# jakub-zarzycki2022/gym-PBN-stac

Measured on NVIDIA B200. Metric: bittner100_env_steps_per_s, higher is better.
Workload: dtype u32

## Files before the change

### gym-pbn-stac_b200/csrc/pbn_b200.cu

```cuda
#include <cmath>
#include <cstdio>
#include <cstdlib>
#include <cstring>
#include <map>
#include <mutex>
#include <string>
#include <type_traits>
#include <vector>

#include "pbn_device.cuh"

static thread_local std::string g_err;
static int fail(int code, const std::string &msg) {
    g_err = msg;
    return code;
}
#define CK(call)                                                                                     \
    do {                                                                                             \
        cudaError_t e_ = (call);                                                                     \
        if (e_ != cudaSuccess) {                                                                     \
            cudaGetLastError();                                                                      \
            return fail(PBN_ERR_CUDA, std::string(#call) + ": " + cudaGetErrorString(e_));           \
        }                                                                                            \
    } while (0)
// ... 1274 lines not shown
    }
    vec_flush_stats(vx, s_stats);
}

template <int MODE>
__global__ void __launch_bounds__(PBN_BLOCK) k_rand_state(NetView nv, DrawView dv, u32 *state, long long B, long long env0) {
    const long long e = (long long)blockIdx.x * blockDim.x + threadIdx.x;
    if (e >= B) return;
    Draw<MODE> d;
    d.init(dv, e, env0 + e);
    u32 acc = 0;
    for (int i = 0; i < nv.n; i++) {
        acc |= (u32)d.randint(0, 2) << (i & 31);
        if ((i & 31) == 31 || i == nv.n - 1) { state[(long long)(i >> 5) * B + e] = acc; acc = 0; }
    }
    d.done(dv, e);
}

__global__ void __launch_bounds__(PBN_BLOCK) k_attractor_index(EnvView ev, int w32, const u32 *state, long long B, int *att_out,
                                                               int staged) {
    const unsigned char *img = staged ? smem_raw : ev.img;
    u32 *sst = reinterpret_cast<u32 *>(smem_raw + index_smem(ev, w32, staged).cols);
    if (staged) stage(smem_raw, ev.img, ev.img_bytes);
    const int *att_off = reinterpret_cast<const int *>(img);
    const u32 *cubes = reinterpret_cast<const u32 *>(img + ev.off_cubes);
    const long long e = (long long)blockIdx.x * PBN_BLOCK + threadIdx.x;
    Col st{sst + threadIdx.x};
    if (e < B) load_state(st, state, B, e, w32);
    __syncthreads();
    if (e >= B) return;
    int idx = -1;
    for (int a = 0; a < ev.n_att && idx < 0; a++)
        if (match_range(cubes, att_off[a], att_off[a + 1], st, w32)) idx = a;
    att_out[e] = idx;
}

__device__ __forceinline__ int ssd_bucket(const SsdParams &sp, const u32 *s_tgt, const Col &st) {
    if (sp.fast_t0 >= 0) {
        u32 field = (*st.wp((u32)sp.fast_t0) >> (sp.fast_t0 & 31)) << (32 - sp.g);
        return (int)__brev(field);
    }
    int b = 0;
    for (int k = 0; k < sp.g; k++) b = (b << 1) | (int)st.bit(s_tgt[k]);
    return b;
}

struct SsdLoopArgs {
    const NetView &nv;
    const EnvView &ev;
    const SsdParams &sp;
    const DrawView &dv;
    const unsigned char *blob;
    const int *att_off;
    const u32 *cubes;
    const u32 *s_tgt;
    u32 *shist;
    unsigned long long *hist;
    u32 *sst;
    int iters;
    u32 nvalid;
    u32 *flipbuf;
    int win;
    long long chain_id;
    unsigned char *coop_buf;
};

__device__ __forceinline__ u32 warp_scan_add(u32 v) {
#pragma unroll
    for (int off = 1; off < 32; off <<= 1)
        asm volatile("{ .reg .pred p; .reg .u32 t; shfl.sync.up.b32 t|p, %0, %1, 0, 0xffffffff; @p add.u32 %0, %0, t; }"
                     : "+r"(v) : "r"(off));
    return v;
}

struct SsdPerturb {
    u32 e0, e1;
    u32 last_p1;
};

__device__ __forceinline__ u32 ssd_gap(u32 word, float inv, float hmd) {
    bool ok;
    u32 gap = geom_gap_approx(word, inv, hmd, &ok);
    if (!ok) gap = geom_gap(word, inv);
    return gap;
}

__device__ __forceinline__ void ssd_round(SsdPerturb &ps, u32 g0, u32 g1) {
    const u32 incl = warp_scan_add(g0 + g1 + 2u);
    ps.e1 = ps.last_p1 - 1u + incl;
    ps.e0 = ps.e1 - 1u - g1;
    ps.last_p1 = __shfl_sync(0xFFFFFFFFu, ps.e1, 31) + 1u;
}

template <bool FULL>
__device__ __forceinline__ void ssd_perturb(SsdPerturb &ps, Draw<PBN_DRAW_PHILOX> &dp, char *warp_cols, u32 W, float inv, float hmd, u32 nvalid) {
    auto apply = [&](u32 &e) {
        if (e < W) {
            const u32 tl = e & 31u;
            if (FULL || tl < nvalid) atomicXor(reinterpret_cast<u32 *>(warp_cols + tl * 4u + ((e >> 10) << 10)), 1u << ((e >> 5) & 31u));
            e = 0xFFFFFFFFu;
        }
    };
    for (;;) {
        apply(ps.e0);
        apply(ps.e1);
        if (ps.last_p1 > W) break;
        const u32 g0 = ssd_gap(dp.next(), inv, hmd);
        const u32 g1 = ssd_gap(dp.next(), inv, hmd);
        ssd_round(ps, g0, g1);
    }
    if (ps.e0 != 0xFFFFFFFFu) ps.e0 -= W;
    if (ps.e1 != 0xFFFFFFFFu) ps.e1 -= W;
    ps.last_p1 -= W;
    __syncwarp();
}

template <bool FULL>
__device__ __forceinline__ void ssd_perturb_buf(SsdPerturb &ps, Draw<PBN_DRAW_PHILOX> &dp, u32 *buf, u32 W, float inv, float hmd, u32 nvalid) {
    auto apply = [&](u32 &e) {
        if (e < W) {
            const u32 tl = e & 31u;
            if (FULL || tl < nvalid) atomicXor(buf + ((e >> 10) << 5) + tl, 1u << ((e >> 5) & 31u));
            e = 0xFFFFFFFFu;
        }
    };
    for (;;) {
        apply(ps.e0);
        apply(ps.e1);
        if (ps.last_p1 > W) break;
        const u32 g0 = ssd_gap(dp.next(), inv, hmd);
        const u32 g1 = ssd_gap(dp.next(), inv, hmd);
        ssd_round(ps, g0, g1);
    }
    if (ps.e0 != 0xFFFFFFFFu) ps.e0 -= W;
    if (ps.e1 != 0xFFFFFFFFu) ps.e1 -= W;
    ps.last_p1 -= W;
}

struct SsdCount {
    int cur;
    u32 run;
};
__device__ __forceinline__ void ssd_count(SsdCount &c, const SsdLoopArgs &a, const Col &st) {
    const int b = ssd_bucket(a.sp, a.s_tgt, st);
    if (b != c.cur) {
        if (a.sp.smem_hist) atomicAdd(&a.shist[c.cur], c.run);
        else atomicAdd(&a.hist[c.cur], (unsigned long long)c.run);
        c.cur = b; c.run = 0;
    }
    c.run++;
}

struct SsdFastPerturb {
    u32 e0, e1, last_p1;
    u32 blk, half, sx, sy;
};

__device__ __forceinline__ void ssd_fast_apply(const SsdFast &f, u32 e) {
    asm volatile("{ .reg .pred p; setp.lt.u32 p, %0, %1; @p red.shared.xor.b32 [%2], %3; }"
                 :: "r"(e), "r"(f.W), "r"((f.warp_cols | ((e << 2) & 0x7Cu)) | (e & 0xFFFFFC00u)),
                    "r"(1u << ((e >> 5) & 31u)) : "memory");
}

__device__ __forceinline__ u32 ssd_fast_gap(const SsdFast &f, u32 word, bool &ok) { return geom_gap_approx(word, f.inv, f.gdelta, &ok); }

__device__ __forceinline__ void ssd_fast_perturb(const SsdFast &f, SsdFastPerturb &ps, const Draw<PBN_DRAW_PHILOX> &dp, const DrawView &dv) {
    ssd_fast_apply(f, ps.e0);
    ssd_fast_apply(f, ps.e1);
    while (ps.last_p1 <= f.W) {
        u32 wa, wb;
        if (ps.half == 0u) {
            u32 x2, x3;
            philox4x32_10_rk(ps.blk, dp.c1, dp.c2, dp.c3, dv, wa, wb, x2, x3);
            ps.blk++;
            ps.sx = x2; ps.sy = x3;
            ps.half = 1u;
        } else {
            wa = ps.sx; wb = ps.sy;
            ps.half = 0u;
        }
        bool ok0, ok1;
        u32 g0 = ssd_fast_gap(f, wa, ok0), g1 = ssd_fast_gap(f, wb, ok1);
        if (!(ok0 && ok1)) {
            if (!ok0) g0 = geom_gap(wa, f.inv);
            if (!ok1) g1 = geom_gap(wb, f.inv);
        }
        const u32 incl = warp_scan_add(g0 + g1 + 2u);
        ps.e1 = ps.last_p1 - 1u + incl;
        ps.e0 = ps.e1 - 1u - g1;
        ps.last_p1 = __reduce_max_sync(0xFFFFFFFFu, ps.e1) + 1u;
        ssd_fast_apply(f, ps.e0);
        ssd_fast_apply(f, ps.e1);
    }
    ps.e0 -= f.W;
    ps.e1 -= f.W;
    ps.last_p1 -= f.W;
    __syncwarp();
}

template <int TQ>
__device__ __forceinline__ int ssd_loop_pred_static(const SsdLoopArgs &a, const Col &st, Draw<PBN_DRAW_PHILOX> &d,
                                                    Draw<PBN_DRAW_PHILOX> &dp, SsdPerturb &ps0, SsdCount &cnt) {
    const NetView &nv = a.nv;
    SsdFast f;
    f.col = keep(smem_addr(st.s));
    f.warp_cols = keep(smem_addr(a.sst + (threadIdx.x & ~31u)));
    f.thr = keep(smem_addr(a.blob + nv.off_thr));
    f.rec = keep(smem_addr(a.blob + nv.off_rec16));
    f.thr_stride = keep((u32)nv.tsq_stride * 16u);
    f.rec_stride = keep((u32)nv.fmax * 16u);
    f.shist = keep(smem_addr(a.shist));
    f.n = keep((u32)nv.n);
    f.W = keep((u32)nv.n * 32u);
    f.b_off = keep(((u32)a.sp.fast_t0 >> 5) << 10);
    f.b_sh = keep((u32)a.sp.fast_t0 & 31u);
    f.b_up = keep(32u - (u32)a.sp.g);
    f.inv = a.sp.inv;
    f.gdelta = 0.5f - a.sp.gdelta;
    SsdFastPerturb ps{ps0.e0, ps0.e1, ps0.last_p1, dp.blk, 0u, 0u, 0u};
    u32 ublk = 0;
    int t = 0;
    u32 cur = (u32)cnt.cur, run = cnt.run;
    auto count = [&]() {
        const u32 b = __brev((lds_u32(f.col + f.b_off) >> f.b_sh) << f.b_up);
        u32 r0;
        asm volatile("{ .reg .pred p; setp.ne.u32 p, %1, %2; @p red.shared.add.u32 [%3], %4; selp.u32 %0, 0, %4, p; }"
                     : "=r"(r0) : "r"(b), "r"(cur), "r"(f.shist + cur * 4u), "r"(run) : "memory");
        cur = b;
        run = r0 + 1u;
    };
    for (int left = a.iters >> 1; left > 0; left--, t += 2) {
        u32 x0, x1, x2, x3;
        philox4x32_10_rk(ublk, d.c1, d.c2, d.c3, a.dv, x0, x1, x2, x3);
        ublk++;
        const FastDraw da = ssd_fast_draw<TQ>(f, x0, x1);
        count();
        ssd_fast_perturb(f, ps, dp, a.dv);
        ssd_fast_apply_update(f, da);
        __syncwarp();
        const FastDraw db = ssd_fast_draw<TQ>(f, x2, x3);
        count();
        ssd_fast_perturb(f, ps, dp, a.dv);
        ssd_fast_apply_update(f, db);
        __syncwarp();
    }
    d.blk = ublk;
    d.have = 0;
    dp.blk = ps.blk;
    dp.have = ps.half ? 2 : 0;
    dp.b0 = ps.sx; dp.b1 = ps.sy;
    ps0.e0 = ps.e0 >= 0x80000000u ? 0xFFFFFFFFu : ps.e0;
    ps0.e1 = ps.e1 >= 0x80000000u ? 0xFFFFFFFFu : ps.e1;
    ps0.last_p1 = ps.last_p1;
    cnt.cur = (int)cur; cnt.run = run;
    return t;
}

template <int NET, int MODE, int TQ, bool HAS_ENV, bool FULL>
__device__ __forceinline__ void ssd_loop(const SsdLoopArgs &a, const Col &st, Draw<MODE> &d, Draw<MODE> &dp) {
    const NetView &nv = a.nv;
    const SsdParams &sp = a.sp;
    const u32 lane = threadIdx.x & 31u;
    const bool active = FULL || lane < a.nvalid;
    const u32 n = (u32)nv.n, W = n * 32u;
    const float inv = sp.inv;
    const float hmd = 0.5f - sp.gdelta;
    const bool flips = inv <= 0.f;
    SsdPerturb ps{0xFFFFFFFFu, 0xFFFFFFFFu, 0u};
    char *warp_cols = reinterpret_cast<char *>(a.sst + (threadIdx.x & ~31u));
    SsdCount cnt{active ? ssd_bucket(sp, a.s_tgt, st) : 0, 0u};
    int t = 0;
    if constexpr (MODE == PBN_DRAW_PHILOX && !HAS_ENV && FULL && NET == PBN_NET_PRED && TQ > 0) {
        if (flips && sp.smem_hist && sp.fast_t0 >= 0 && nv.off_rec16) t = ssd_loop_pred_static<TQ>(a, st, d, dp, ps, cnt);
    }
    if constexpr (MODE == PBN_DRAW_PHILOX && !HAS_ENV && FULL) {
        u32 ublk = d.blk;
        for (; t + 1 < a.iters; t += 2) {
            u32 x0, x1, x2, x3;
            philox4x32_10(ublk, d.c1, d.c2, d.c3, d.k0, d.k1, x0, x1, x2, x3);
            ublk++;
            ssd_count(cnt, a, st);
            if (flips) ssd_perturb<true>(ps, dp, warp_cols, W, inv, hmd, 32u);
            micro_step_words<NET, TQ>(nv, a.blob, st, x0, x1, d);
            __syncwarp();
            ssd_count(cnt, a, st);
            if (flips) ssd_perturb<true>(ps, dp, warp_cols, W, inv, hmd, 32u);
            micro_step_words<NET, TQ>(nv, a.blob, st, x2, x3, d);
            __syncwarp();
        }
        d.blk = ublk;
        d.have = 0;
    }
    if constexpr (MODE == PBN_DRAW_PHILOX && HAS_ENV) {
        if (a.flipbuf != nullptr && !a.ev.force) {
            const int w32 = nv.w32;
            u32 *fb = a.flipbuf + (size_t)(threadIdx.x >> 5) * a.win * w32 * 32;
            u32 pos = 0;
            while (t < a.iters) {
                const int kk = a.iters - t < a.win ? a.iters - t : a.win;
                for (int k = 0; k < kk; k++) {
                    for (int w = 0; w < w32; w++) fb[(k * w32 + w) * 32 + lane] = 0u;
                    __syncwarp();
                    if (flips) ssd_perturb_buf<FULL>(ps, dp, fb + k * w32 * 32, W, inv, hmd, a.nvalid);
                }
                __syncwarp();
                int k = 0, in = 0;
                bool start = true;
                for (;;) {
                    const bool live = active && k < kk;
                    if (!__any_sync(0xFFFFFFFFu, live)) break;
                    if (live) {
                        if (start) {
                            ssd_count(cnt, a, st);
                            for (int w = 0; w < w32; w++) st.set_word(w, st.word(w) ^ fb[(k * w32 + w) * 32 + lane]);
                            micro_step<NET, MODE, TQ>(nv, a.blob, st, d);
                            in = 1;
                            pos++;
                            start = false;
                        } else if (in >= a.ev.max_inner || is_attracting(a.ev, a.att_off, a.cubes, st, w32)) {
                            k++;
                            start = true;
                        } else {
                            micro_step<NET, MODE, TQ>(nv, a.blob, st, d);
                            in++;
                            pos++;
                        }
                    }
                    if constexpr (NET == PBN_NET_PRED) {
                        const unsigned hv = __ballot_sync(0xFFFFFFFFu, live && !start && k < kk);
                        if (hv != 0u && __popc(__ballot_sync(0xFFFFFFFFu, active && k < kk)) <= PBN_COOP_MAX) {
                            const u32 base = pos - (u32)in;
                            const int v = w32 == 1 ? coop_take_over<TQ, true>(hv, nv, a.ev, a.dv, a.blob, a.att_off, a.cubes, a.sst, a.coop_buf,
                                                                              a.chain_id, in, base, a.ev.max_inner, 32)
                                                   : coop_take_over<TQ, false>(hv, nv, a.ev, a.dv, a.blob, a.att_off, a.cubes, a.sst, a.coop_buf,
                                                                               a.chain_id, in, base, a.ev.max_inner, 32);
                            if (v != in) {
                                pos += (u32)(v - in);
                                in = v;
                                d.seek(a.dv, 0, a.chain_id, 2u * pos, 0u);
                            }
                        }
                    }
                }
                __syncwarp();
                t += kk;
            }
        }
    }
    for (; t < a.iters; t++) {
        if (active) ssd_count(cnt, a, st);
        if constexpr (MODE == PBN_DRAW_REPLAY) {
            if (active)
                for (u32 j = 0; j < n; j++)
                    if (d.dbl() < sp.p) st.flip(j);
        } else {
            if (flips) ssd_perturb<FULL>(ps, dp, warp_cols, W, inv, hmd, a.nvalid);
        }
        if (active) {
            micro_step<NET, MODE, TQ>(nv, a.blob, st, d);
            if constexpr (HAS_ENV) {
                if (!a.ev.force) {
                    int in = 1;
                    while (in < a.ev.max_inner && !is_attracting(a.ev, a.att_off, a.cubes, st, nv.w32)) {
                        micro_step<NET, MODE, TQ>(nv, a.blob, st, d);
                        in++;
                    }
                }
            }
        }
        if constexpr (MODE == PBN_DRAW_PHILOX) __syncwarp();
    }
    if (active && cnt.run) {
        if (sp.smem_hist) atomicAdd(&a.shist[cnt.cur], cnt.run);
        else atomicAdd(&a.hist[cnt.cur], (unsigned long long)cnt.run);
    }
}

#ifndef PBN_SSD_MIN_BLOCKS
#define PBN_SSD_MIN_BLOCKS 4
#endif
template <int NET, int MODE, int TQ, bool HAS_ENV>
__global__ void __launch_bounds__(PBN_BLOCK, HAS_ENV ? 3 : PBN_SSD_MIN_BLOCKS) k_ssd(NetView nv, EnvView ev, DrawView dv, SsdParams sp, u32 *state,
                                                   long long chains, long long env0, int iters,
                                                   unsigned long long *hist) {
    unsigned char *blob = smem_raw;
    const SsdSmem L = ssd_smem(nv, ev, sp, HAS_ENV);
    unsigned char *img = smem_raw + L.img;
    u32 *s_tgt = reinterpret_cast<u32 *>(smem_raw + L.tgt);
    u32 *shist = reinterpret_cast<u32 *>(smem_raw + L.hist);
    const int nb = 1 << sp.g;
    u32 *sst = align_cols(shist + (sp.smem_hist ? nb : 0), nv.w32);
    stage(blob, nv.blob, L.image);
    if (HAS_ENV) stage(img, ev.img, ev.img_bytes);
    if (threadIdx.x == 0) {
#pragma unroll
        for (int k = 0; k < 24; k++) s_tgt[k] = (u32)sp.tgt[k];
    }
    if (sp.smem_hist)
        for (int b = threadIdx.x; b < nb; b += PBN_BLOCK) shist[b] = 0;
    const int *att_off = reinterpret_cast<const int *>(img);
    const u32 *cubes = reinterpret_cast<const u32 *>(img + ev.off_cubes);
    const long long e = (long long)blockIdx.x * PBN_BLOCK + threadIdx.x;
    const int w32 = nv.w32;
    Col st{sst + threadIdx.x};
    const int win = sp.win;
    u32 *flipbuf = (HAS_ENV && win > 0) ? sst + L.flip : nullptr;
// ... 312 lines not shown

extern "C" int pbn_env_step_f64(const PbnEnv *env, uint32_t *state, int32_t *n_steps, const int32_t *target_att,
                                const int32_t *actions, int32_t K, uint32_t *obs_state, int32_t *reward, double *reward_f64,
                                uint8_t *terminated, uint8_t *truncated, int32_t *inner_steps, int64_t B, int64_t env0,
                                const PbnDraws *draws, void *stream) {
    if (!reward_f64) return fail(PBN_ERR_ARG, "reward_f64 is null");
    return env_step_impl(env, state, n_steps, target_att, actions, K, obs_state, reward, terminated, truncated, inner_steps, B,
                         env0, draws, nullptr, stream, reward_f64);
}

extern "C" int pbn_vec_step(const PbnEnv *env, uint32_t *state, int32_t *n_steps, int32_t *target_att, const int32_t *actions,
                            int32_t K, uint32_t *obs_state, int32_t *reward, uint8_t *terminated, uint8_t *truncated,
                            int32_t *inner_steps, const PbnVecState *vec, int64_t B, int64_t env0, const PbnDraws *draws,
                            void *stream) {
    if (!vec) return fail(PBN_ERR_ARG, "vec is null");
    return env_step_impl(env, state, n_steps, target_att, actions, K, obs_state, reward, terminated, truncated, inner_steps, B,
                         env0, draws, vec, stream);
}

extern "C" int pbn_env_step_plan(const PbnEnv *env, uint32_t *state, int32_t *n_steps, int32_t *target_att, const int32_t *actions,
                                 int32_t K, uint32_t *obs_state, int32_t *reward, uint8_t *terminated, uint8_t *truncated,
                                 int32_t *inner_steps, const PbnVecState *vec, const PbnStepPlan *plan, int64_t B, int64_t env0,
                                 const PbnDraws *draws, void *stream) {
    if (!plan) return fail(PBN_ERR_ARG, "plan is null");
    return env_step_impl(env, state, n_steps, target_att, actions, K, obs_state, reward, terminated, truncated, inner_steps, B,
                         env0, draws, vec, stream, nullptr, plan);
}

static int env_reset_impl(const PbnEnv *env, uint32_t *state, int32_t *n_steps, int32_t *target_att, uint32_t *target_state,
                          const uint8_t *mask, int64_t B, int64_t env0, const PbnDraws *draws, void *stream, CurView cv);
extern "C" int pbn_env_reset(const PbnEnv *env, uint32_t *state, int32_t *n_steps, int32_t *target_att, uint32_t *target_state,
                             const uint8_t *mask, int64_t B, int64_t env0, const PbnDraws *draws, void *stream) {
    return env_reset_impl(env, state, n_steps, target_att, target_state, mask, B, env0, draws, stream, CurView{nullptr, nullptr, 0});
}
extern "C" int pbn_env_reset_cur(const PbnEnv *env, uint32_t *state, int32_t *n_steps, int32_t *target_att, uint32_t *target_state,
                                 const uint8_t *mask, double *probabilities, int32_t *pair_ids, int32_t sample_pair, int64_t B,
                                 int64_t env0, const PbnDraws *draws, void *stream) {
    if (!env || !probabilities || !pair_ids) return fail(PBN_ERR_ARG, "bad argument");
    if (env->v.kind != PBN_ENV_MULTI || env->v.n_att < 2 || env->v.n_att > 64)
        return fail(PBN_ERR_ARG, "a probability table needs a MULTI env with 2..64 attractors");
    if (!draws || draws->mode != PBN_DRAW_PHILOX) return fail(PBN_ERR_UNSUPPORTED, "the curriculum draws its pairs from Philox words");
    return env_reset_impl(env, state, n_steps, target_att, target_state, mask, B, env0, draws, stream,
                          CurView{probabilities, pair_ids, sample_pair != 0});
}
static int env_reset_impl(const PbnEnv *env, uint32_t *state, int32_t *n_steps, int32_t *target_att, uint32_t *target_state,
                          const uint8_t *mask, int64_t B, int64_t env0, const PbnDraws *draws, void *stream, CurView cv) {
    if (!env || !state || B < 0) return fail(PBN_ERR_ARG, "bad argument");
    const EnvView &ev = env->v;
    if (ev.kind == PBN_ENV_TARGET || ev.kind == PBN_ENV_MULTI) {
        if (!n_steps || !target_att) return fail(PBN_ERR_ARG, "target envs need n_steps and target_att");
        if (ev.n_att < (ev.kind == PBN_ENV_TARGET ? 2 : 1)) return fail(PBN_ERR_ARG, "reset needs attractors (sample of 2, pbn_target.py:333)");
    } else {
        if (ev.n_att < 1) return fail(PBN_ERR_ARG, "reset needs attractors");
        if (!env->has_small_att) return fail(PBN_ERR_ARG, "reset needs an attractor with at most 10 states (pbn_env.py:196-199 would loop forever)");
    }
    if (int rc = check_draws(draws)) return rc;
    if (B == 0) return PBN_OK;
    const DrawView dv = make_draws(draws);
    const unsigned grid = (unsigned)((B + PBN_BLOCK - 1) / PBN_BLOCK);
    cudaStream_t s = (cudaStream_t)stream;
    if (dv.mode == PBN_DRAW_PHILOX)
        k_env_reset<PBN_DRAW_PHILOX><<<grid, PBN_BLOCK, 0, s>>>(env->net->v, ev, dv, state, n_steps, target_att, target_state, mask, B, env0, cv);
    else
        k_env_reset<PBN_DRAW_REPLAY><<<grid, PBN_BLOCK, 0, s>>>(env->net->v, ev, dv, state, n_steps, target_att, target_state, mask, B, env0, cv);
    CK(cudaGetLastError());
    return PBN_OK;
}

extern "C" int pbn_rand_state(const PbnNet *net, uint32_t *state, int64_t B, int64_t env0, const PbnDraws *draws, void *stream) {
    if (!net || !state || B < 0) return fail(PBN_ERR_ARG, "bad argument");
    if (int rc = check_draws(draws)) return rc;
    if (B == 0) return PBN_OK;
    const DrawView dv = make_draws(draws);
    const unsigned grid = (unsigned)((B + PBN_BLOCK - 1) / PBN_BLOCK);
    cudaStream_t s = (cudaStream_t)stream;
    if (dv.mode == PBN_DRAW_PHILOX) k_rand_state<PBN_DRAW_PHILOX><<<grid, PBN_BLOCK, 0, s>>>(net->v, dv, state, B, env0);
    else k_rand_state<PBN_DRAW_REPLAY><<<grid, PBN_BLOCK, 0, s>>>(net->v, dv, state, B, env0);
    CK(cudaGetLastError());
    return PBN_OK;
}

extern "C" int pbn_env_attractor_index(const PbnEnv *env, const uint32_t *state, int64_t B, int32_t *att_out, void *stream) {
    if (!env || !state || !att_out || B < 0) return fail(PBN_ERR_ARG, "bad argument");
    const EnvView &ev = env->v;
    if (ev.n_att < 1) return fail(PBN_ERR_ARG, "the env has no attractor list");
    if (B == 0) return PBN_OK;
    const int w32 = env->net->v.w32;
    const unsigned grid = (unsigned)((B + PBN_BLOCK - 1) / PBN_BLOCK);
    const int staged = index_smem(ev, w32, true).bytes <= 64 * 1024;
    const size_t smem = index_smem(ev, w32, staged).bytes;
    if (int rc = fit_smem(k_attractor_index, "k_attractor_index", smem)) return rc;
    k_attractor_index<<<grid, PBN_BLOCK, smem, (cudaStream_t)stream>>>(ev, w32, state, B, att_out, staged);
    CK(cudaGetLastError());
    return PBN_OK;
}

__global__ void __launch_bounds__(256) k_geom_verify(float inv, float dlt, unsigned int *bad, unsigned int *taken) {
    const u32 r = ((u32)blockIdx.x * 256u + threadIdx.x) << 9;
    bool ok;
    const u32 a = geom_gap_approx(r, inv, 0.5f - dlt, &ok);
    if (ok) {
        if (a != geom_gap(r, inv)) atomicAdd(bad, 1u);
    } else {
        atomicAdd(taken, 1u);
    }
}
static float geom_shortcut_delta(float inv, cudaStream_t s) {
    static std::mutex mu;
    static std::map<std::pair<int, u32>, float> cache;
    if (!(inv < 0.f)) return 1.0f;
    const float dlt = -inv * 2.0f * (24.0f * 2.3841858e-7f + 2e-7f);
    if (!(dlt < 0.05f)) return 1.0f;
    int dev = 0;
    cudaGetDevice(&dev);
    u32 bits;
    memcpy(&bits, &inv, 4);
    std::lock_guard<std::mutex> lk(mu);
    auto it = cache.find({dev, bits});
    if (it != cache.end()) return it->second;
    cudaStreamCaptureStatus cap = cudaStreamCaptureStatusNone;
    if (cudaStreamIsCapturing(s, &cap) != cudaSuccess || cap != cudaStreamCaptureStatusNone) return 1.0f;
    unsigned int *d = nullptr, h[2] = {1u, 0u};
    float res = 1.0f;
    if (cudaMalloc(&d, 8) == cudaSuccess) {
        if (cudaMemsetAsync(d, 0, 8, s) == cudaSuccess) {
            k_geom_verify<<<(1u << 23) / 256u, 256, 0, s>>>(inv, dlt, d, d + 1);
            if (cudaMemcpyAsync(h, d, 8, cudaMemcpyDeviceToHost, s) == cudaSuccess && cudaStreamSynchronize(s) == cudaSuccess &&
                h[0] == 0u)
                res = dlt;
        }
        cudaFree(d);
    }
    cache[{dev, bits}] = res;
    return res;
}

extern "C" int pbn_geom_shortcut_check(double p, float *delta, uint32_t *disagree, uint32_t *fallback) {
    if (!(p > 0.0 && p < 1.0) || !delta || !disagree || !fallback) return fail(PBN_ERR_ARG, "bad argument");
    const float inv = (float)(1.0 / std::log2(1.0 - p));
    *delta = geom_shortcut_delta(inv, nullptr);
    const float dlt = -inv * 2.0f * (24.0f * 2.3841858e-7f + 2e-7f);
    unsigned int *d = nullptr, h[2] = {0u, 0u};
    CK(cudaMalloc(&d, 8));
    cudaMemset(d, 0, 8);
    k_geom_verify<<<(1u << 23) / 256u, 256>>>(inv, dlt < 0.5f ? dlt : 0.5f, d, d + 1);
    cudaError_t e = cudaMemcpy(h, d, 8, cudaMemcpyDeviceToHost);
    cudaFree(d);
    CK(e);
    *disagree = h[0];
    *fallback = h[1];
    return PBN_OK;
}

extern "C" int pbn_ssd(const PbnNet *net, const PbnEnv *env, uint32_t *state, int64_t chains, int64_t env0, int64_t iters,
                       double p, const int32_t *tgt, int32_t g, uint64_t *hist, const PbnDraws *draws, void *stream) {
    if (!net || !state || !tgt || !hist || chains < 0 || iters < 0) return fail(PBN_ERR_ARG, "bad argument");
    if (g < 1 || g > 24) return fail(PBN_ERR_ARG, "1 <= g <= 24 target nodes");
    if (!(p >= 0.0 && p <= 1.0)) return fail(PBN_ERR_ARG, "Invalid Bit Flip Probability value.");
    if (env && env->net != net) return fail(PBN_ERR_ARG, "env belongs to another network");
    if (int rc = check_draws(draws)) return rc;
    if (chains == 0 || iters == 0) return PBN_OK;
    if (draws->mode == PBN_DRAW_PHILOX && p > 0 && (env0 & 31))
        return fail(PBN_ERR_ARG, "env0 must be a multiple of 32: the perturbation stream is shared by groups of 32 consecutive chain ids");
    if (p > 0 && p < 1e-6) return fail(PBN_ERR_UNSUPPORTED, "bit_flip_prob below 1e-6 is not supported (gap law is truncated at 2^25)");
    const NetView &nv = net->v;
    const DrawView dv = make_draws(draws);
    SsdParams sp;
    sp.g = g; sp.p = p; sp.smem_hist = g <= 12;
    sp.inv = p <= 0 ? 1.0f : (p >= 1 ? 0.0f : (float)(1.0 / std::log2(1.0 - p)));
    sp.gdelta = 1.0f;
    memset(sp.tgt, 0, sizeof sp.tgt);
    for (int k = 0; k < g; k++) {
        if (tgt[k] < 0 || tgt[k] >= nv.n) return fail(PBN_ERR_ARG, "target node out of range");
        if (tgt[k] > 32767) return fail(PBN_ERR_UNSUPPORTED, "target node indices above 32767 are not supported");
        sp.tgt[k] = (short)tgt[k];
    }
    sp.fast_t0 = tgt[0];
    for (int k = 1; k < g; k++)
        if (tgt[k] != tgt[0] + k) sp.fast_t0 = -1;
    if (sp.fast_t0 >= 0 && (tgt[0] >> 5) != ((tgt[0] + g - 1) >> 5)) sp.fast_t0 = -1;
    if (iters >= (1LL << 31) || (sp.smem_hist && (double)iters * PBN_BLOCK >= 4294967296.0))
        return fail(PBN_ERR_ARG, "iters too large for one launch; split the estimate");
    const unsigned grid = (unsigned)((chains + PBN_BLOCK - 1) / PBN_BLOCK);
    EnvView ev;
    memset(&ev, 0, sizeof ev);
    if (env) ev = env->v;
    sp.win = (env && draws->mode == PBN_DRAW_PHILOX && !ev.force && nv.w32 <= 8) ? (16 / nv.w32 > 2 ? 16 / nv.w32 : 2) : 0;
    const size_t smem = ssd_smem(nv, ev, sp, env != nullptr).bytes;
    cudaStream_t s = (cudaStream_t)stream;
    if (draws->mode == PBN_DRAW_PHILOX) sp.gdelta = geom_shortcut_delta(sp.inv, s);
    auto launch = [&](auto kernel) -> int {
        if (int rc = fit_smem(kernel, "k_ssd", smem)) return rc;
        kernel<<<grid, PBN_BLOCK, smem, s>>>(nv, ev, dv, sp, state, chains, env0, (int)iters, (unsigned long long *)hist);
        CK(cudaGetLastError());
        return PBN_OK;
    };
    return dispatch(nv.kind, dv.mode, nv.ts, [&](auto NK, auto MD, auto TQ) {
        return env ? launch(k_ssd<NK, MD, TQ, true>) : launch(k_ssd<NK, MD, TQ, false>);
    });
}

struct HistParams { int g; short tgt[24]; };
__global__ void __launch_bounds__(256) k_bucket_hist(const u32 *state, long long B, HistParams hp, unsigned long long *hist) {
    extern __shared__ u32 sh[];
    const int nb = 1 << hp.g;
    const bool smem = hp.g <= 12;
    if (smem)
        for (int b = threadIdx.x; b < nb; b += blockDim.x) sh[b] = 0;
    __syncthreads();
    for (long long e = (long long)blockIdx.x * blockDim.x + threadIdx.x; e < B; e += (long long)gridDim.x * blockDim.x) {
        int b = 0;
#pragma unroll
        for (int k = 0; k < 24; k++)
            if (k < hp.g) b = (b << 1) | (int)((state[(long long)(hp.tgt[k] >> 5) * B + e] >> (hp.tgt[k] & 31)) & 1u);
        if (smem) atomicAdd(&sh[b], 1u);
        else atomicAdd(&hist[b], 1ULL);
    }
    if (smem) {
        __syncthreads();
        for (int b = threadIdx.x; b < nb; b += blockDim.x)
            if (sh[b]) atomicAdd(&hist[b], (unsigned long long)sh[b]);
    }
}
extern "C" int pbn_bucket_hist(const uint32_t *state, int64_t B, int32_t n_nodes, const int32_t *tgt, int32_t g, uint64_t *hist,
                               void *stream) {
    if (!state || !tgt || !hist || B < 0 || n_nodes < 1) return fail(PBN_ERR_ARG, "bad argument");
    if (g < 1 || g > 24) return fail(PBN_ERR_ARG, "1 <= g <= 24 target nodes");
    if (B == 0) return PBN_OK;
    HistParams hp;
    memset(&hp, 0, sizeof hp);
    hp.g = g;
    for (int k = 0; k < g; k++) {
        if (tgt[k] < 0 || tgt[k] >= n_nodes) return fail(PBN_ERR_ARG, "target node out of range");
        hp.tgt[k] = (short)tgt[k];
    }
    long long blocks = (B + 255) / 256;
    if (blocks > 148 * 8) blocks = 148 * 8;
    k_bucket_hist<<<(unsigned)blocks, 256, g <= 12 ? ((size_t)4 << g) : 0, (cudaStream_t)stream>>>(state, B, hp, (unsigned long long *)hist);
    CK(cudaGetLastError());
    return PBN_OK;
}

extern "C" int pbn_ssd_host(const PbnNet *net, const PbnEnv *env, int64_t chains, int64_t env0, int64_t iters, double p,
                            const int32_t *tgt, int32_t g, uint64_t seed, uint32_t epoch, uint64_t *hist_host) {
    if (!net || !hist_host || chains < 1) return fail(PBN_ERR_ARG, "bad argument");
    if (g < 1 || g > 24) return fail(PBN_ERR_ARG, "1 <= g <= 24 target nodes");
    u32 *state = nullptr;
    uint64_t *hist = nullptr;
    CK(cudaMalloc(&state, (size_t)net->v.w32 * chains * 4));
    CK(cudaMalloc(&hist, (size_t)8 << g));
    CK(cudaMemsetAsync(hist, 0, (size_t)8 << g, 0));
    PbnDraws d;
    memset(&d, 0, sizeof d);
    d.mode = PBN_DRAW_PHILOX; d.seed = seed; d.epoch = epoch;
    int rc = pbn_rand_state(net, state, chains, env0, &d, nullptr);
    d.epoch = epoch + 1;
    if (!rc) rc = pbn_ssd(net, env, state, chains, env0, iters, p, tgt, g, hist, &d, nullptr);
    if (!rc) {
        cudaError_t e = cudaMemcpy(hist_host, hist, (size_t)8 << g, cudaMemcpyDeviceToHost);
        if (e != cudaSuccess) rc = fail(PBN_ERR_CUDA, cudaGetErrorString(e));
    }
    cudaFree(state);
    cudaFree(hist);
    return rc;
}

__global__ void __launch_bounds__(256) k_change_masks(NetView nv, u32 *masks) {
    const unsigned long long total = 1ULL << nv.n;
    for (unsigned long long s = (unsigned long long)blockIdx.x * blockDim.x + threadIdx.x; s < total;
         s += (unsigned long long)gridDim.x * blockDim.x) {
        const u32 st = (u32)s;
        u32 m = 0;
        if (nv.kind == PBN_NET_TT) {
            const uint2 *node = reinterpret_cast<const uint2 *>(nv.blob + nv.off_node);
            const unsigned short *in = reinterpret_cast<const unsigned short *>(nv.blob + nv.off_in);
            for (int i = 0; i < nv.n; i++) {
                const uint2 nr = node[i];
                const int k = (int)(nr.y >> 16);
                u32 idx = 0;
                for (int q = 0; q < k; q++) idx = (idx << 1) | ((st >> in[(nr.y & 0xFFFF) + q]) & 1u);
                const double p = nv.tt_prob[nr.x + idx];
                const u32 cur = (st >> i) & 1u;
                if ((cur == 0 && p > 0.0) || (cur == 1 && p < 1.0)) m |= 1u << i;
            }
        } else {
            const uint2 *rec = reinterpret_cast<const uint2 *>(nv.blob + nv.off_rec);
            for (int i = 0; i < nv.n; i++) {
                const int q0 = nv.pr_off[i], f = nv.pr_off[i + 1] - q0;
                const u32 cur = (st >> i) & 1u;
                bool can = false;
                double prev = 0.0;
                for (int j = 0; j < f; j++) {
                    const double c = nv.pr_cum[q0 + j];
                    if (c > prev) {
                        const uint2 r = rec[i * nv.fmax + j];
                        const u32 idx = (((st >> (r.x & 0xFF)) & 1u) << 3) | (((st >> ((r.x >> 8) & 0xFF)) & 1u) << 2) |
                                        (((st >> ((r.x >> 16) & 0xFF)) & 1u) << 1) | ((st >> (r.x >> 24)) & 1u);
                        can |= (((r.y >> idx) & 1u) != cur);
                    }
                    prev = c;
                }
                if (can) m |= 1u << i;
            }
        }
        masks[s] = m;
    }
}

__global__ void __launch_bounds__(256) k_stg_expand(const u32 *masks, int n, const u32 *frontier, const u32 *visited,
                                                    const u32 *within, u32 *next, int direction) {
    const unsigned long long words = (1ULL << n) >> 5 ? (1ULL << n) >> 5 : 1ULL;
    for (unsigned long long w = (unsigned long long)blockIdx.x * blockDim.x + threadIdx.x; w < words;
         w += (unsigned long long)gridDim.x * blockDim.x) {
        u32 fw = frontier[w];
        while (fw) {
            const int b = __ffs(fw) - 1;
            fw &= fw - 1;
            const u32 s = (u32)(w << 5) | (u32)b;
            if (direction == 0) {
                u32 m = masks[s];
                while (m) {
                    const int i = __ffs(m) - 1;
                    m &= m - 1;
// ... 115 lines not shown
```

### gym-pbn-stac_b200/csrc/pbn_smem.cuh

```cuda
#pragma once

struct SsdParams {
    int g;
    int smem_hist;
    int fast_t0;
    int win;
    float inv;
    float gdelta;
    double p;
    short tgt[24];
};

struct Smem {
    size_t image = 0, bytes = 0;
    __host__ __device__ size_t add(size_t n) { const size_t at = bytes; bytes += n; return at; }
};
struct RolloutSmem : Smem { size_t cols; };
__host__ __device__ inline RolloutSmem rollout_smem(const NetView &nv, bool sync) {
    RolloutSmem L;
    L.bytes = L.image = sync ? nv.blob_bytes : nv.blob_fast_bytes;
    L.cols = L.add(col_align_bytes(nv.w32) + (size_t)2 * nv.w32 * PBN_BLOCK * 4);
    return L;
}
struct SlicedSmem : Smem { size_t lm, words; };
__host__ __device__ inline SlicedSmem sliced_smem(const NetView &nv) {
    SlicedSmem L;
    L.bytes = L.image = nv.blob_bytes;
    L.lm = L.add((size_t)nv.n * (nv.fmax * 16 + 4) * 4);
    L.words = L.add((size_t)(PBN_BLOCK / 32) * 2 * nv.w32 * 32 * 4);
    return L;
}
struct EnvSmem : Smem {
    size_t img, cols;
    int coop;
};
__host__ __device__ inline EnvSmem env_smem(const NetView &nv, const EnvView &ev, int ncols, bool fast, bool coop) {
    EnvSmem L;
    L.bytes = L.image = fast ? nv.blob_fast_bytes : nv.blob_bytes;
    L.img = L.add(ev.img_bytes);
    L.coop = ncols * nv.w32 * PBN_BLOCK;
    L.cols = L.add((fast ? col_align_bytes(nv.w32) : 0) + (size_t)L.coop * 4);
    L.add(coop ? (size_t)(PBN_BLOCK / 32) * coop_warp_bytes(nv.w32) : 0);
    return L;
}
struct IndexSmem : Smem { size_t cols; };
__host__ __device__ inline IndexSmem index_smem(const EnvView &ev, int w32, bool staged) {
    IndexSmem L;
    L.add(staged ? ev.img_bytes : 0);
    L.cols = L.add((size_t)w32 * PBN_BLOCK * 4);
    return L;
}
struct SsdSmem : Smem {
    size_t img, tgt, hist, cols;
    int flip, coop;
};
__host__ __device__ inline SsdSmem ssd_smem(const NetView &nv, const EnvView &ev, const SsdParams &sp, bool env) {
    SsdSmem L;
    L.bytes = L.image = env ? nv.blob_bytes : nv.blob_fast_bytes;
    L.img = L.add(env ? ev.img_bytes : 0);
    L.tgt = L.add(32 * 4);
    L.hist = L.add((size_t)(sp.smem_hist ? 1 << sp.g : 0) * 4);
    L.flip = nv.w32 * PBN_BLOCK;
    L.coop = (PBN_BLOCK / 32) * sp.win * nv.w32 * 32;
    const size_t coop = sp.win ? (size_t)(PBN_BLOCK / 32) * coop_warp_bytes(nv.w32) : 0;
    L.cols = L.add(col_align_bytes(nv.w32) + ((size_t)L.flip + L.coop) * 4 + coop);
    return L;
}
```

Before: 166.1 billion.

## Precompute perturbation flip slots with due-step scheduling instead of per-step window rebasing

Perturbation flip positions are converted once, via a magic-number division by the window size, into a due iteration plus a precomputed shared-memory address and bit mask. Each step then issues an unconditional red.xor whose mask is zero unless the slot is due. The gap-generation loop runs only on the step where the next window begins. This removes the per-step subtract-and-compare and the loop check, at the cost of more registers and a reconstruction step that converts the slots back to positions on exit.

Measured after the change: 173.6 billion, median of 6. 4.5% higher.

```diff
diff --git a/gym-pbn-stac_b200/csrc/pbn_b200.cu b/gym-pbn-stac_b200/csrc/pbn_b200.cu
--- a/gym-pbn-stac_b200/csrc/pbn_b200.cu
+++ b/gym-pbn-stac_b200/csrc/pbn_b200.cu
@@ -1450,55 +1450,70 @@
 }
 
 struct SsdFastPerturb {
-    u32 e0, e1, last_p1;
+    u32 t0, t1;
+    u32 a0, a1;
+    u32 m0, m1;
+    u32 next;
+    u32 last_p1;
     u32 blk, half, sx, sy;
 };
 
-__device__ __forceinline__ void ssd_fast_apply(const SsdFast &f, u32 e) {
-    asm volatile("{ .reg .pred p; setp.lt.u32 p, %0, %1; @p red.shared.xor.b32 [%2], %3; }"
-                 :: "r"(e), "r"(f.W), "r"((f.warp_cols | ((e << 2) & 0x7Cu)) | (e & 0xFFFFFC00u)),
-                    "r"(1u << ((e >> 5) & 31u)) : "memory");
+__device__ __forceinline__ void ssd_fast_apply(u32 t_due, u32 a, u32 m, u32 it) { red_xor_u32(a, t_due == it ? m : 0u); }
+
+__device__ __forceinline__ void ssd_fast_slot(const SsdFast &f, const SsdParams &sp, u32 e, u32 it, u32 &t_due, u32 &a, u32 &m) {
+    const u32 q = __umulhi(e >> 4, sp.wq_mul) >> sp.wq_sh;
+    const u32 c = e - q * f.W;
+    t_due = it + q;
+    a = f.warp_cols | ((c << 2) & 0x7Cu) | (c & 0xFFFFFC00u);
+    m = 1u << ((c >> 5) & 31u);
 }
 
 __device__ __forceinline__ u32 ssd_fast_gap(const SsdFast &f, u32 word, bool &ok) { return geom_gap_approx(word, f.inv, f.gdelta, &ok); }
 
-__device__ __forceinline__ void ssd_fast_perturb(const SsdFast &f, SsdFastPerturb &ps, const Draw<PBN_DRAW_PHILOX> &dp, const DrawView &dv) {
-    ssd_fast_apply(f, ps.e0);
-    ssd_fast_apply(f, ps.e1);
-    while (ps.last_p1 <= f.W) {
-        u32 wa, wb;
-        if (ps.half == 0u) {
-            u32 x2, x3;
-            philox4x32_10_rk(ps.blk, dp.c1, dp.c2, dp.c3, dv, wa, wb, x2, x3);
-            ps.blk++;
-            ps.sx = x2; ps.sy = x3;
-            ps.half = 1u;
-        } else {
-            wa = ps.sx; wb = ps.sy;
-            ps.half = 0u;
-        }
-        bool ok0, ok1;
-        u32 g0 = ssd_fast_gap(f, wa, ok0), g1 = ssd_fast_gap(f, wb, ok1);
-        if (!(ok0 && ok1)) {
-            if (!ok0) g0 = geom_gap(wa, f.inv);
-            if (!ok1) g1 = geom_gap(wb, f.inv);
-        }
-        const u32 incl = warp_scan_add(g0 + g1 + 2u);
-        ps.e1 = ps.last_p1 - 1u + incl;
-        ps.e0 = ps.e1 - 1u - g1;
-        ps.last_p1 = __reduce_max_sync(0xFFFFFFFFu, ps.e1) + 1u;
-        ssd_fast_apply(f, ps.e0);
-        ssd_fast_apply(f, ps.e1);
-    }
-    ps.e0 -= f.W;
-    ps.e1 -= f.W;
-    ps.last_p1 -= f.W;
+__device__ __forceinline__ void ssd_fast_perturb(const SsdFast &f, const SsdParams &sp, SsdFastPerturb &ps, const Draw<PBN_DRAW_PHILOX> &dp,
+                                                 const DrawView &dv, u32 it) {
+    ssd_fast_apply(ps.t0, ps.a0, ps.m0, it);
+    ssd_fast_apply(ps.t1, ps.a1, ps.m1, it);
+    if (ps.next == it) {
+        u32 last_p1 = ps.last_p1;
+        do {
+            u32 wa, wb;
+            if (ps.half == 0u) {
+                u32 x2, x3;
+                philox4x32_10_rk(ps.blk, dp.c1, dp.c2, dp.c3, dv, wa, wb, x2, x3);
+                ps.blk++;
+                ps.sx = x2; ps.sy = x3;
+                ps.half = 1u;
+            } else {
+                wa = ps.sx; wb = ps.sy;
+                ps.half = 0u;
+            }
+            bool ok0, ok1;
+            u32 g0 = ssd_fast_gap(f, wa, ok0), g1 = ssd_fast_gap(f, wb, ok1);
+            if (!(ok0 && ok1)) {
+                if (!ok0) g0 = geom_gap(wa, f.inv);
+                if (!ok1) g1 = geom_gap(wb, f.inv);
+            }
+            const u32 incl = warp_scan_add(g0 + g1 + 2u);
+            const u32 e1 = last_p1 - 1u + incl;
+            const u32 e0 = e1 - 1u - g1;
+            last_p1 = __reduce_max_sync(0xFFFFFFFFu, e1) + 1u;
+            ssd_fast_slot(f, sp, e0, it, ps.t0, ps.a0, ps.m0);
+            ssd_fast_slot(f, sp, e1, it, ps.t1, ps.a1, ps.m1);
+            ssd_fast_apply(ps.t0, ps.a0, ps.m0, it);
+            ssd_fast_apply(ps.t1, ps.a1, ps.m1, it);
+        } while (last_p1 <= f.W);
+        const u32 q = __umulhi((last_p1 - 1u) >> 4, sp.wq_mul) >> sp.wq_sh;
+        ps.next = it + q;
+        ps.last_p1 = last_p1 - q * f.W;
+    }
     __syncwarp();
 }
 
 template <int TQ>
 __device__ __forceinline__ int ssd_loop_pred_static(const SsdLoopArgs &a, const Col &st, Draw<PBN_DRAW_PHILOX> &d,
                                                     Draw<PBN_DRAW_PHILOX> &dp, SsdPerturb &ps0, SsdCount &cnt) {
+    if (a.iters < 2) return 0;
     const NetView &nv = a.nv;
     SsdFast f;
     f.col = keep(smem_addr(st.s));
@@ -1515,7 +1530,7 @@
     f.b_up = keep(32u - (u32)a.sp.g);
     f.inv = a.sp.inv;
     f.gdelta = 0.5f - a.sp.gdelta;
-    SsdFastPerturb ps{ps0.e0, ps0.e1, ps0.last_p1, dp.blk, 0u, 0u, 0u};
+    SsdFastPerturb ps{~0u, ~0u, f.warp_cols, f.warp_cols, 0u, 0u, 0u, ps0.last_p1, dp.blk, 0u, 0u, 0u};
     u32 ublk = 0;
     int t = 0;
     u32 cur = (u32)cnt.cur, run = cnt.run;
@@ -1533,12 +1548,12 @@
         ublk++;
         const FastDraw da = ssd_fast_draw<TQ>(f, x0, x1);
         count();
-        ssd_fast_perturb(f, ps, dp, a.dv);
+        ssd_fast_perturb(f, a.sp, ps, dp, a.dv, (u32)t);
         ssd_fast_apply_update(f, da);
         __syncwarp();
         const FastDraw db = ssd_fast_draw<TQ>(f, x2, x3);
         count();
-        ssd_fast_perturb(f, ps, dp, a.dv);
+        ssd_fast_perturb(f, a.sp, ps, dp, a.dv, (u32)t + 1u);
         ssd_fast_apply_update(f, db);
         __syncwarp();
     }
@@ -1547,9 +1562,15 @@
     dp.blk = ps.blk;
     dp.have = ps.half ? 2 : 0;
     dp.b0 = ps.sx; dp.b1 = ps.sy;
-    ps0.e0 = ps.e0 >= 0x80000000u ? 0xFFFFFFFFu : ps.e0;
-    ps0.e1 = ps.e1 >= 0x80000000u ? 0xFFFFFFFFu : ps.e1;
-    ps0.last_p1 = ps.last_p1;
+    const u32 tu = (u32)t;
+    auto position = [&](u32 t_due, u32 addr, u32 m) {
+        if (t_due < tu) return 0xFFFFFFFFu;
+        const u32 x = addr ^ f.warp_cols;
+        return (t_due - tu) * f.W + ((x & 0xFFFFFC00u) | ((31u - __clz(m)) << 5) | ((x >> 2) & 31u));
+    };
+    ps0.e0 = position(ps.t0, ps.a0, ps.m0);
+    ps0.e1 = position(ps.t1, ps.a1, ps.m1);
+    ps0.last_p1 = (ps.next - tu) * f.W + ps.last_p1;
     cnt.cur = (int)cur; cnt.run = run;
     return t;
 }
@@ -2168,6 +2189,12 @@
     return PBN_OK;
 }
 
+static void ssd_window_div(int n, SsdParams &sp) {
+    const unsigned long long d = 2ull * (unsigned)n;
+    sp.wq_sh = 63 - __builtin_clzll(d - 1);
+    sp.wq_mul = (unsigned)(((1ull << (32 + sp.wq_sh)) + d - 1) / d);
+}
+
 extern "C" int pbn_ssd(const PbnNet *net, const PbnEnv *env, uint32_t *state, int64_t chains, int64_t env0, int64_t iters,
                        double p, const int32_t *tgt, int32_t g, uint64_t *hist, const PbnDraws *draws, void *stream) {
     if (!net || !state || !tgt || !hist || chains < 0 || iters < 0) return fail(PBN_ERR_ARG, "bad argument");
@@ -2185,6 +2212,7 @@
     sp.g = g; sp.p = p; sp.smem_hist = g <= 12;
     sp.inv = p <= 0 ? 1.0f : (p >= 1 ? 0.0f : (float)(1.0 / std::log2(1.0 - p)));
     sp.gdelta = 1.0f;
+    ssd_window_div(nv.n, sp);
     memset(sp.tgt, 0, sizeof sp.tgt);
     for (int k = 0; k < g; k++) {
         if (tgt[k] < 0 || tgt[k] >= nv.n) return fail(PBN_ERR_ARG, "target node out of range");
diff --git a/gym-pbn-stac_b200/csrc/pbn_smem.cuh b/gym-pbn-stac_b200/csrc/pbn_smem.cuh
--- a/gym-pbn-stac_b200/csrc/pbn_smem.cuh
+++ b/gym-pbn-stac_b200/csrc/pbn_smem.cuh
@@ -7,6 +7,8 @@
     int win;
     float inv;
     float gdelta;
+    unsigned wq_mul;
+    int wq_sh;
     double p;
     short tgt[24];
 };
```
